# asarigun/mma

Hardware: AMD Instinct MI355X
Metric: aggregated edges/sec (fwd+bwd) MultiMaskConv (higher is better)
Workload: dtype f32

## Files before the change

### include/mma_amd.h

```cpp
#ifndef MMA_AMD_H
#define MMA_AMD_H

#include <stdint.h>

#ifdef __cplusplus
extern "C" {
#endif

#define MMA_ABI_VERSION 40
#define MMA_MAX_K 8

enum {
  MMA_KIND_SUM = 0,
  MMA_KIND_MEAN = 1,
  MMA_KIND_MAX = 2,
  MMA_KIND_MIN = 3,
  MMA_KIND_SOFTMAX = 4,
  MMA_KIND_SOFTMIN = 5
};
enum { MMA_ACT_SIGMOID = 0, MMA_ACT_RAW = 1 };

enum { MMA_DROP_NONE = 0, MMA_DROP_HASH = 1, MMA_DROP_EXPLICIT = 2 };

int mma_abi_version(void);
// ... 161 lines not shown
int mma_gemm_f16x2_k256p_h(const void* Ap, const int32_t* sce, const void* Bt2, const float* col_unscale, uint16_t* C, int64_t ldc,
                           int64_t M, int32_t N, void* stream);
int mma_gemm_f16x2_n128(const float* A, int64_t lda, const float* row_max, const void* Bt2, const float* col_unscale,
                        float* C, int64_t ldc, int64_t M, int32_t K, int32_t accumulate, void* stream);
int mma_gemm_f16x2_nlp(const float* A, int64_t lda, const float* row_max, const void* Bt2, const float* col_unscale,
                       float* C, int64_t ldc, int64_t M, int32_t N, int32_t K, int32_t accumulate, void* stream);
int64_t mma_gemm_bf16x3_tn_workspace_floats(int64_t M, int32_t KA, int32_t NC);
int mma_gemm_bf16x3_tn(const float* X, int64_t ldx, const float* G, int64_t ldg, float* C, float* ws, int64_t ws_floats,
                       int64_t M, int32_t KA, int32_t NC, void* stream);
int64_t mma_gemm_bf16x3_tn_batched_workspace_floats(int64_t M, int32_t KA, int32_t NC, int32_t B);
int mma_gemm_bf16x3_tn_batched(const float* X, int64_t ldx, int64_t xb, const float* G, int64_t ldg, int64_t gb, float* C, float* ws,
                               int64_t ws_floats, int64_t M, int32_t KA, int32_t NC, int32_t B, void* stream);
int64_t mma_gemm_f16x2_tn_workspace_floats(int64_t M, int32_t KA, int32_t NC);
int mma_gemm_f16x2_tn(const float* X, int64_t ldx, const float* G, int64_t ldg, const float* x_row_max, const float* g_row_max,
                      float* C, float* ws, int64_t ws_floats, int64_t M, int32_t KA, int32_t NC, void* stream);

int mma_pack_rows(const float* src, int64_t lds, const int32_t* idx, int64_t n_idx,
                  float* dst, int64_t ldd, int32_t width, void* stream);
int mma_unpack_add_rows(const float* src, int64_t lds, const int32_t* idx, int64_t n_idx,
                        float* dst, int64_t ldd, int32_t width, void* stream);
int mma_unpack_add_rows_csr(const float* src, int64_t lds, const int32_t* rows, const int32_t* segptr, const int32_t* pos,
                            int64_t n_rows, float* dst, int64_t ldd, int32_t width, void* stream);

int64_t mma_col_sum_workspace_floats(int64_t R, int32_t C);
int mma_col_sum(const float* g, int64_t ldg, int64_t R, int32_t C, float* out, float* ws, int64_t ws_floats,
                void* stream);

int64_t mma_tower_linear_bwd_blocks(int64_t N);
int mma_tower_linear_bwd(const float* gy, const float* a, const float* W, float* ga, float* part, int64_t n_blocks,
                         int64_t N, int32_t T, int32_t O, int32_t C, void* stream);
// ... 103 lines not shown
```

### mma_amd/_abi.py

```python
ABI_VERSION = 40
FUNCTIONS = {
    "mma_abi_version": ("int", []),
    "mma_last_error": ("const char*", []),
    "mma_build_stamp": ("const char*", []),
    "mma_nc_fused_fwd": ("int", [("T", "T", "x"), ("i", "i64", "ldx"), ("T", "T", "P"), ("i", "i64", "ldp"), ("T", "T", "Q"), ("i", "i64", "ldq"), ("T", "T", "rowptr"), ("T", "T", "col"), ("T", "T", "items"), ("i", "i64", "n_items"), ("i", "i64", "n_wave_items"), ("T", "T", "hubs"), ("i", "i64", "n_hubs"), ("T", "T", "partial"), ("i", "i64", "n_slots"), ("T", "T", "m"), ("T", "T", "m_sum"), ("i", "i64", "ldms"), ("T", "T", "T"), ("T", "T", "sel"), ("i", "i64", "ldt"), ("T", "T", "crow"), ("i", "i64", "ldc"), ("i", "i64", "N"), ("i", "i64", "E"), ("i", "i32", "H"), ("i", "i32", "K"), ("H", "H", "kind_host"), ("H", "H", "act_host"), ("i", "i32", "drop_mode"), ("i", "u32", "drop_thr"), ("i", "u64", "seed"), ("T", "T", "seed_dev"), ("i", "i64", "drop_edge_base"), ("T", "T", "keep"), ("T", "T", "sync"), ("S", "S", "stream")]),
    "mma_nc_bwd_node": ("int", [("T", "T", "g"), ("i", "i64", "g_kstride"), ("i", "i64", "ldgr"), ("T", "T", "sel"), ("T", "T", "T"), ("i", "i64", "ldt"), ("T", "T", "rowptr"), ("T", "T", "gs"), ("i", "i64", "ldgs"), ("T", "T", "crow"), ("i", "i64", "ldc"), ("T", "T", "gP"), ("i", "i64", "ldgp"), ("T", "T", "gxs"), ("i", "i64", "ldgx"), ("T", "T", "row_max"), ("i", "i64", "N"), ("i", "i32", "H"), ("i", "i32", "K"), ("H", "H", "kind_host"), ("S", "S", "stream")]),
    "mma_nc_crow_floats": ("int64_t", [("i", "i32", "H"), ("i", "i32", "K"), ("H", "H", "kind_host")]),
    "mma_nc_fused_bwd": ("int", [("T", "T", "x"), ("i", "i64", "ldx"), ("T", "T", "P"), ("i", "i64", "ldp"), ("T", "T", "Q"), ("i", "i64", "ldq"), ("T", "T", "gs"), ("i", "i64", "ldg"), ("T", "T", "g"), ("i", "i64", "ldgg"), ("T", "T", "crow"), ("i", "i64", "ldc"), ("H", "H", "kind_host"), ("T", "T", "gxs"), ("i", "i64", "ldgx"), ("T", "T", "T"), ("i", "i64", "ldt"), ("T", "T", "gP"), ("i", "i64", "ldgp"), ("i", "i64", "n_targets"), ("T", "T", "t_col"), ("T", "T", "t_eid"), ("T", "T", "items"), ("i", "i64", "n_items"), ("i", "i64", "n_wave_items"), ("T", "T", "hubs"), ("i", "i64", "n_hubs"), ("T", "T", "partial"), ("i", "i64", "n_slots"), ("T", "T", "gQ"), ("i", "i64", "ldgq"), ("T", "T", "gx"), ("i", "i64", "ldgxo"), ("T", "T", "row_max"), ("i", "i64", "N"), ("i", "i64", "E"), ("i", "i32", "H"), ("i", "i32", "K"), ("H", "H", "act_host"), ("i", "i32", "drop_mode"), ("i", "u32", "drop_thr"), ("i", "u64", "seed"), ("T", "T", "seed_dev"), ("i", "i64", "drop_edge_base"), ("T", "T", "keep"), ("T", "T", "sync"), ("S", "S", "stream")]),
    "mma_nc_fused_fwd_h": ("int", [("T", "T", "x"), ("i", "i64", "ldx"), ("T", "T", "P"), ("i", "i64", "ldp"), ("T", "T", "Q"), ("i", "i64", "ldq"), ("T", "T", "rowptr"), ("T", "T", "col"), ("T", "T", "items"), ("i", "i64", "n_items"), ("i", "i64", "n_wave_items"), ("T", "T", "hubs"), ("i", "i64", "n_hubs"), ("T", "T", "partial"), ("i", "i64", "n_slots"), ("T", "T", "m"), ("T", "T", "m_sum"), ("i", "i64", "ldms"), ("T", "T", "T"), ("T", "T", "sel"), ("i", "i64", "ldt"), ("T", "T", "crow"), ("i", "i64", "ldc"), ("i", "i64", "N"), ("i", "i64", "E"), ("i", "i32", "H"), ("i", "i32", "K"), ("H", "H", "kind_host"), ("H", "H", "act_host"), ("i", "i32", "drop_mode"), ("i", "u32", "drop_thr"), ("i", "u64", "seed"), ("T", "T", "seed_dev"), ("i", "i64", "drop_edge_base"), ("T", "T", "keep"), ("T", "T", "sync"), ("S", "S", "stream")]),
    "mma_nc_fused_bwd_h": ("int", [("T", "T", "x"), ("i", "i64", "ldx"), ("T", "T", "P"), ("i", "i64", "ldp"), ("T", "T", "Q"), ("i", "i64", "ldq"), ("T", "T", "gs"), ("i", "i64", "ldg"), ("T", "T", "g"), ("i", "i64", "ldgg"), ("T", "T", "crow"), ("i", "i64", "ldc"), ("H", "H", "kind_host"), ("T", "T", "gxs"), ("i", "i64", "ldgx"), ("T", "T", "T"), ("i", "i64", "ldt"), ("T", "T", "gP"), ("i", "i64", "ldgp"), ("i", "i64", "n_targets"), ("T", "T", "t_col"), ("T", "T", "t_eid"), ("T", "T", "items"), ("i", "i64", "n_items"), ("i", "i64", "n_wave_items"), ("T", "T", "hubs"), ("i", "i64", "n_hubs"), ("T", "T", "partial"), ("i", "i64", "n_slots"), ("T", "T", "gQ"), ("i", "i64", "ldgq"), ("T", "T", "gx"), ("i", "i64", "ldgxo"), ("T", "T", "row_max"), ("i", "i64", "N"), ("i", "i64", "E"), ("i", "i32", "H"), ("i", "i32", "K"), ("H", "H", "act_host"), ("i", "i32", "drop_mode"), ("i", "u32", "drop_thr"), ("i", "u64", "seed"), ("T", "T", "seed_dev"), ("i", "i64", "drop_edge_base"), ("T", "T", "keep"), ("T", "T", "sync"), ("S", "S", "stream")]),
    "mma_rows_to_bf16": ("int", [("T", "T", "src"), ("i", "i64", "lds"), ("T", "T", "dst"), ("i", "i64", "ldd"), ("i", "i64", "rows"), ("i", "i64", "cols"), ("S", "S", "stream")]),
    "mma_nc_std_fwd": ("int", [("T", "T", "x"), ("i", "i64", "ldx"), ("T", "T", "P"), ("i", "i64", "ldp"), ("T", "T", "Q"), ("i", "i64", "ldq"), ("T", "T", "rowptr"), ("T", "T", "col"), ("T", "T", "items"), ("i", "i64", "n_items"), ("i", "i64", "n_wave_items"), ("T", "T", "hubs"), ("i", "i64", "n_hubs"), ("T", "T", "partial"), ("i", "i64", "n_slots"), ("T", "T", "m"), ("i", "i64", "ldms"), ("T", "T", "saved"), ("i", "i64", "ldt"), ("i", "i64", "N"), ("i", "i64", "E"), ("i", "i32", "H"), ("H", "H", "act_host"), ("i", "i32", "drop_mode"), ("i", "u32", "drop_thr"), ("i", "u64", "seed"), ("T", "T", "seed_dev"), ("i", "i64", "drop_edge_base"), ("T", "T", "keep"), ("S", "S", "stream")]),
    "mma_nc_std_bwd": ("int", [("T", "T", "x"), ("i", "i64", "ldx"), ("T", "T", "P"), ("i", "i64", "ldp"), ("T", "T", "Q"), ("i", "i64", "ldq"), ("T", "T", "g"), ("i", "i64", "ldg"), ("T", "T", "saved"), ("i", "i64", "ldt"), ("T", "T", "gr"), ("i", "i64", "ldgr"), ("T", "T", "gP"), ("i", "i64", "ldgp"), ("i", "i64", "n_targets"), ("T", "T", "t_col"), ("T", "T", "t_eid"), ("T", "T", "items"), ("i", "i64", "n_items"), ("i", "i64", "n_wave_items"), ("T", "T", "hubs"), ("i", "i64", "n_hubs"), ("T", "T", "partial"), ("i", "i64", "n_slots"), ("T", "T", "gQ"), ("i", "i64", "ldgq"), ("T", "T", "gx"), ("i", "i64", "ldgx"), ("i", "i64", "N"), ("i", "i64", "E"), ("i", "i32", "H"), ("H", "H", "act_host"), ("i", "i32", "drop_mode"), ("i", "u32", "drop_thr"), ("i", "u64", "seed"), ("T", "T", "seed_dev"), ("i", "i64", "drop_edge_base"), ("T", "T", "keep"), ("S", "S", "stream")]),
    "mma_nc_std_fwd_h": ("int", [("T", "T", "x"), ("i", "i64", "ldx"), ("T", "T", "P"), ("i", "i64", "ldp"), ("T", "T", "Q"), ("i", "i64", "ldq"), ("T", "T", "rowptr"), ("T", "T", "col"), ("T", "T", "items"), ("i", "i64", "n_items"), ("i", "i64", "n_wave_items"), ("T", "T", "hubs"), ("i", "i64", "n_hubs"), ("T", "T", "partial"), ("i", "i64", "n_slots"), ("T", "T", "m"), ("i", "i64", "ldms"), ("T", "T", "saved"), ("i", "i64", "ldt"), ("i", "i64", "N"), ("i", "i64", "E"), ("i", "i32", "H"), ("H", "H", "act_host"), ("i", "i32", "drop_mode"), ("i", "u32", "drop_thr"), ("i", "u64", "seed"), ("T", "T", "seed_dev"), ("i", "i64", "drop_edge_base"), ("T", "T", "keep"), ("S", "S", "stream")]),
    "mma_nc_std_bwd_h": ("int", [("T", "T", "x"), ("i", "i64", "ldx"), ("T", "T", "P"), ("i", "i64", "ldp"), ("T", "T", "Q"), ("i", "i64", "ldq"), ("T", "T", "g"), ("i", "i64", "ldg"), ("T", "T", "saved"), ("i", "i64", "ldt"), ("T", "T", "gr"), ("i", "i64", "ldgr"), ("T", "T", "gP"), ("i", "i64", "ldgp"), ("i", "i64", "n_targets"), ("T", "T", "t_col"), ("T", "T", "t_eid"), ("T", "T", "items"), ("i", "i64", "n_items"), ("i", "i64", "n_wave_items"), ("T", "T", "hubs"), ("i", "i64", "n_hubs"), ("T", "T", "partial"), ("i", "i64", "n_slots"), ("T", "T", "gQ"), ("i", "i64", "ldgq"), ("T", "T", "gx"), ("i", "i64", "ldgx"), ("i", "i64", "N"), ("i", "i64", "E"), ("i", "i32", "H"), ("H", "H", "act_host"), ("i", "i32", "drop_mode"), ("i", "u32", "drop_thr"), ("i", "u64", "seed"), ("T", "T", "seed_dev"), ("i", "i64", "drop_edge_base"), ("T", "T", "keep"), ("S", "S", "stream")]),
    "mma_csr_spmm": ("int", [("T", "T", "rowptr"), ("T", "T", "col"), ("T", "T", "val"), ("T", "T", "B"), ("i", "i64", "ldb"), ("i", "i64", "rows_per_block"), ("i", "i32", "K"), ("T", "T", "bias"), ("T", "T", "out"), ("i", "i64", "ldo"), ("i", "i64", "n_rows"), ("i", "i32", "C"), ("S", "S", "stream")]),
    "mma_csr_spmm_rm": ("int", [("T", "T", "rowptr"), ("T", "T", "col"), ("T", "T", "val"), ("T", "T", "B"), ("i", "i64", "ldb"), ("i", "i64", "rows_per_block"), ("i", "i32", "K"), ("T", "T", "bias"), ("T", "T", "out"), ("i", "i64", "ldo"), ("i", "i64", "n_rows"), ("i", "i32", "C"), ("T", "T", "row_max"), ("S", "S", "stream")]),
    "mma_csr_spmm_items": ("int", [("T", "T", "col"), ("T", "T", "val"), ("T", "T", "B"), ("i", "i64", "ldb"), ("T", "T", "bias"), ("T", "T", "out"), ("i", "i64", "ldo"), ("T", "T", "items"), ("i", "i64", "n_items"), ("i", "i64", "n_wave_items"), ("T", "T", "hubs"), ("i", "i64", "n_hubs"), ("T", "T", "partial"), ("i", "i64", "n_slots"), ("i", "i32", "C"), ("S", "S", "stream")]),
    "mma_split_bf16x3": ("int", [("T", "T", "in"), ("i", "i64", "n"), ("T", "T", "out_3n_bf16"), ("S", "S", "stream")]),
    "mma_gemm_bf16x3": ("int", [("T", "T", "A"), ("i", "i64", "lda"), ("T", "T", "Bt3"), ("T", "T", "C"), ("i", "i64", "ldc"), ("i", "i64", "M"), ("i", "i32", "N"), ("i", "i32", "K"), ("i", "i32", "accumulate"), ("S", "S", "stream")]),
    "mma_row_absmax": ("int", [("T", "T", "A"), ("i", "i64", "lda"), ("i", "i64", "M"), ("i", "i32", "cols"), ("T", "T", "out"), ("S", "S", "stream")]),
    "mma_split_f16x2": ("int", [("T", "T", "w"), ("i", "i64", "stride_k"), ("i", "i64", "stride_n"), ("i", "i32", "K"), ("i", "i32", "N"), ("T", "T", "bt2"), ("T", "T", "col_unscale"), ("i", "i32", "plain_lo"), ("S", "S", "stream")]),
    "mma_gemm_f16x2": ("int", [("T", "T", "A"), ("i", "i64", "lda"), ("T", "T", "Bt2"), ("T", "T", "col_unscale"), ("T", "T", "C"), ("i", "i64", "ldc"), ("T", "T", "a_row_max"), ("i", "i64", "M"), ("i", "i32", "N"), ("S", "S", "stream")]),
    "mma_gemm_f16x2_k": ("int", [("T", "T", "A"), ("i", "i64", "lda"), ("T", "T", "Bt2"), ("T", "T", "col_unscale"), ("T", "T", "C"), ("i", "i64", "ldc"), ("T", "T", "a_row_max"), ("i", "i64", "M"), ("i", "i32", "N"), ("i", "i32", "K"), ("S", "S", "stream")]),
    "mma_gemm_f16x2_k256": ("int", [("T", "T", "A"), ("i", "i64", "lda"), ("T", "T", "row_max"), ("T", "T", "Bt2"), ("T", "T", "col_unscale"), ("T", "T", "C"), ("i", "i64", "ldc"), ("i", "i64", "M"), ("i", "i32", "N"), ("S", "S", "stream")]),
    "mma_pack_f16x2_k256_bytes": ("int64_t", [("i", "i64", "M")]),
    "mma_pack_f16x2_k256": ("int", [("T", "T", "A"), ("i", "i64", "lda"), ("i", "i64", "M"), ("T", "T", "Ap"), ("T", "T", "sce"), ("T", "T", "row_max"), ("S", "S", "stream")]),
    "mma_gemm_f16x2_k256p": ("int", [("T", "T", "Ap"), ("T", "T", "sce"), ("T", "T", "Bt2"), ("T", "T", "col_unscale"), ("T", "T", "C"), ("i", "i64", "ldc"), ("i", "i64", "M"), ("i", "i32", "N"), ("S", "S", "stream")]),
    "mma_gemm_f16x2_k_h": ("int", [("T", "T", "A"), ("i", "i64", "lda"), ("T", "T", "Bt2"), ("T", "T", "col_unscale"), ("T", "T", "C"), ("i", "i64", "ldc"), ("T", "T", "a_row_max"), ("i", "i64", "M"), ("i", "i32", "N"), ("i", "i32", "K"), ("S", "S", "stream")]),
    "mma_gemm_f16x2_k256_h": ("int", [("T", "T", "A"), ("i", "i64", "lda"), ("T", "T", "row_max"), ("T", "T", "Bt2"), ("T", "T", "col_unscale"), ("T", "T", "C"), ("i", "i64", "ldc"), ("i", "i64", "M"), ("i", "i32", "N"), ("S", "S", "stream")]),
    "mma_gemm_f16x2_k256p_h": ("int", [("T", "T", "Ap"), ("T", "T", "sce"), ("T", "T", "Bt2"), ("T", "T", "col_unscale"), ("T", "T", "C"), ("i", "i64", "ldc"), ("i", "i64", "M"), ("i", "i32", "N"), ("S", "S", "stream")]),
    "mma_gemm_f16x2_n128": ("int", [("T", "T", "A"), ("i", "i64", "lda"), ("T", "T", "row_max"), ("T", "T", "Bt2"), ("T", "T", "col_unscale"), ("T", "T", "C"), ("i", "i64", "ldc"), ("i", "i64", "M"), ("i", "i32", "K"), ("i", "i32", "accumulate"), ("S", "S", "stream")]),
    "mma_gemm_f16x2_nlp": ("int", [("T", "T", "A"), ("i", "i64", "lda"), ("T", "T", "row_max"), ("T", "T", "Bt2"), ("T", "T", "col_unscale"), ("T", "T", "C"), ("i", "i64", "ldc"), ("i", "i64", "M"), ("i", "i32", "N"), ("i", "i32", "K"), ("i", "i32", "accumulate"), ("S", "S", "stream")]),
    "mma_gemm_bf16x3_tn_workspace_floats": ("int64_t", [("i", "i64", "M"), ("i", "i32", "KA"), ("i", "i32", "NC")]),
    "mma_gemm_bf16x3_tn": ("int", [("T", "T", "X"), ("i", "i64", "ldx"), ("T", "T", "G"), ("i", "i64", "ldg"), ("T", "T", "C"), ("T", "T", "ws"), ("i", "i64", "ws_floats"), ("i", "i64", "M"), ("i", "i32", "KA"), ("i", "i32", "NC"), ("S", "S", "stream")]),
    "mma_gemm_bf16x3_tn_batched_workspace_floats": ("int64_t", [("i", "i64", "M"), ("i", "i32", "KA"), ("i", "i32", "NC"), ("i", "i32", "B")]),
    "mma_gemm_bf16x3_tn_batched": ("int", [("T", "T", "X"), ("i", "i64", "ldx"), ("i", "i64", "xb"), ("T", "T", "G"), ("i", "i64", "ldg"), ("i", "i64", "gb"), ("T", "T", "C"), ("T", "T", "ws"), ("i", "i64", "ws_floats"), ("i", "i64", "M"), ("i", "i32", "KA"), ("i", "i32", "NC"), ("i", "i32", "B"), ("S", "S", "stream")]),
    "mma_gemm_f16x2_tn_workspace_floats": ("int64_t", [("i", "i64", "M"), ("i", "i32", "KA"), ("i", "i32", "NC")]),
    "mma_gemm_f16x2_tn": ("int", [("T", "T", "X"), ("i", "i64", "ldx"), ("T", "T", "G"), ("i", "i64", "ldg"), ("T", "T", "x_row_max"), ("T", "T", "g_row_max"), ("T", "T", "C"), ("T", "T", "ws"), ("i", "i64", "ws_floats"), ("i", "i64", "M"), ("i", "i32", "KA"), ("i", "i32", "NC"), ("S", "S", "stream")]),
    "mma_pack_rows": ("int", [("T", "T", "src"), ("i", "i64", "lds"), ("T", "T", "idx"), ("i", "i64", "n_idx"), ("T", "T", "dst"), ("i", "i64", "ldd"), ("i", "i32", "width"), ("S", "S", "stream")]),
    "mma_unpack_add_rows": ("int", [("T", "T", "src"), ("i", "i64", "lds"), ("T", "T", "idx"), ("i", "i64", "n_idx"), ("T", "T", "dst"), ("i", "i64", "ldd"), ("i", "i32", "width"), ("S", "S", "stream")]),
    "mma_unpack_add_rows_csr": ("int", [("T", "T", "src"), ("i", "i64", "lds"), ("T", "T", "rows"), ("T", "T", "segptr"), ("T", "T", "pos"), ("i", "i64", "n_rows"), ("T", "T", "dst"), ("i", "i64", "ldd"), ("i", "i32", "width"), ("S", "S", "stream")]),
    "mma_col_sum_workspace_floats": ("int64_t", [("i", "i64", "R"), ("i", "i32", "C")]),
    "mma_col_sum": ("int", [("T", "T", "g"), ("i", "i64", "ldg"), ("i", "i64", "R"), ("i", "i32", "C"), ("T", "T", "out"), ("T", "T", "ws"), ("i", "i64", "ws_floats"), ("S", "S", "stream")]),
    "mma_tower_linear_bwd_blocks": ("int64_t", [("i", "i64", "N")]),
    "mma_tower_linear_bwd": ("int", [("T", "T", "gy"), ("T", "T", "a"), ("T", "T", "W"), ("T", "T", "ga"), ("T", "T", "part"), ("i", "i64", "n_blocks"), ("i", "i64", "N"), ("i", "i32", "T"), ("i", "i32", "O"), ("i", "i32", "C"), ("S", "S", "stream")]),
    "mma_tower_post_kfp": ("int64_t", [("i", "i32", "KF")]),
    "mma_tower_post_weights": ("int", [("T", "T", "Wo"), ("i", "i32", "T"), ("i", "i32", "O"), ("i", "i32", "S"), ("i", "i32", "KF"), ("T", "T", "Wa"), ("T", "T", "Wb"), ("S", "S", "stream")]),
    "mma_skinny_linear_weights": ("int", [("T", "T", "W"), ("i", "i32", "O"), ("i", "i32", "K"), ("T", "T", "Wa"), ("T", "T", "Wb"), ("S", "S", "stream")]),
    "mma_tower_post_gw_reduce": ("int", [("T", "T", "part"), ("i", "i64", "n_chunks"), ("i", "i32", "T"), ("i", "i32", "S"), ("i", "i32", "O"), ("i", "i32", "KF"), ("T", "T", "gWo"), ("S", "S", "stream")]),
    "mma_tower_post_fits": ("int", [("i", "i32", "KF"), ("i", "i32", "S")]),
    "mma_tower_post_pre": ("int", [("T", "T", "rowptr"), ("T", "T", "pre"), ("i", "i64", "N"), ("i", "i32", "S"), ("H", "H", "scaler_host"), ("f", "f32", "avg_log"), ("f", "f32", "avg_lin"), ("S", "S", "stream")]),
    "mma_tower_post_fwd": ("int", [("T", "T", "agg"), ("i", "i64", "lda"), ("T", "T", "pre"), ("T", "T", "Wa"), ("T", "T", "y"), ("i", "i64", "ldy"), ("i", "i64", "N"), ("i", "i32", "T"), ("i", "i32", "KF"), ("i", "i32", "S"), ("i", "i32", "O"), ("H", "H", "scaler_host"), ("f", "f32", "avg_log"), ("f", "f32", "avg_lin"), ("S", "S", "stream")]),
    "mma_tower_post_bwd": ("int", [("T", "T", "gy"), ("i", "i64", "ldg"), ("T", "T", "pre"), ("T", "T", "Wb"), ("T", "T", "gagg"), ("i", "i64", "lda"), ("T", "T", "gys"), ("i", "i64", "ldgs"), ("i", "i64", "N"), ("i", "i32", "T"), ("i", "i32", "KF"), ("i", "i32", "S"), ("i", "i32", "O"), ("H", "H", "scaler_host"), ("f", "f32", "avg_log"), ("f", "f32", "avg_lin"), ("S", "S", "stream")]),
# ... 30 lines not shown
```

### mma_amd/csrc/gemm_x3.hip

```cpp
#include <algorithm>
#include <cstdlib>
#include "common.h"

#ifndef MMA_ABL
#define MMA_ABL 0
#endif

namespace mma {

constexpr int kAbl = MMA_ABL;

typedef __attribute__((ext_vector_type(8))) __bf16 bf16x8;
typedef __attribute__((ext_vector_type(16))) float f32x16;

constexpr int kKC = 128;
constexpr int kKCPersist = 64;
struct GemmParams {
  const float* A; int64_t lda;
  const __bf16* Bt;
  float* C; int64_t ldc;
  int64_t M; int N, K;
  int accumulate;
};

// ... 1254 lines not shown
  if (wave_active) {
    float* out = p.part + (size_t)split * (p.part_ss ? (size_t)p.part_ss : (size_t)p.KA * p.NC) + (size_t)bz * p.KA * p.NC +
                 (size_t)wave * 32 * p.NC + gcol0 + r31;
#pragma unroll
    for (int ct = 0; ct < 4; ++ct) {
      if (ct < n_ct) {
#pragma unroll
        for (int r = 0; r < 16; ++r)
          if (FULLCT || (wave * 32 + acc_row(r) + 4 * h < p.KA && gcol0 + ct * 32 + r31 < p.NC))
            out[(size_t)(acc_row(r) + 4 * h) * p.NC + ct * 32] = acc[ct][r];
      }
    }
  }
}

typedef __attribute__((ext_vector_type(4))) unsigned int u32x4;
constexpr int kTn2Slab = 2 * kTnPiece;
constexpr int kTnMaxSpread = 40;

__global__ void tn_state_init_kernel(int* state) {
  if (threadIdx.x < 4) state[threadIdx.x] = 0;
}

__global__ __launch_bounds__(256) void tn_scale_range_kernel(const float* xmax, const float* gmax, int64_t M, int* state) {
  __shared__ int red[3][4];
  int hi = 0, lo = 0, bad = 0;
  for (int64_t i = (int64_t)blockIdx.x * blockDim.x + threadIdx.x; i < M; i += (int64_t)gridDim.x * blockDim.x) {
    const uint32_t xb = __float_as_uint(xmax[i]) & 0x7fffffffu, gb = __float_as_uint(gmax[i]) & 0x7fffffffu;
    if (xb != 0 && gb != 0) {
      const int ex = (int)(xb >> 23), eg = (int)(gb >> 23);
      if (ex == 255 || eg == 255 || ex == 0 || eg == 0) bad = 1;
      else { const int t = ex + eg - 254; hi = max(hi, t + 1024); lo = max(lo, 1024 - t); }
    }
  }
#pragma unroll
  for (int o = 32; o > 0; o >>= 1) {
    hi = max(hi, __shfl_xor(hi, o, 64)); lo = max(lo, __shfl_xor(lo, o, 64)); bad |= __shfl_xor(bad, o, 64);
  }
  const int wave = threadIdx.x >> 6;
  if ((threadIdx.x & 63) == 0) { red[0][wave] = hi; red[1][wave] = lo; red[2][wave] = bad; }
  __syncthreads();
  if (threadIdx.x == 0) {
    hi = max(max(red[0][0], red[0][1]), max(red[0][2], red[0][3]));
    lo = max(max(red[1][0], red[1][1]), max(red[1][2], red[1][3]));
    bad = red[2][0] | red[2][1] | red[2][2] | red[2][3];
    if (hi) atomicMax(state + 0, hi);
    if (lo) atomicMax(state + 1, lo);
    if (bad) atomicOr(state + 2, 1);
  }
}

__global__ void tn_scale_rows_kernel(const float* xmax, const float* gmax, int64_t M, int64_t M_pad, int* state, uint16_t* sxh,
                                     uint16_t* sgh) {
  const int64_t i = (int64_t)blockIdx.x * blockDim.x + threadIdx.x;
  const int T = state[0] ? state[0] - 1024 : 28;
  if (i == 0) state[3] = T - 28;
  const uint32_t xb = i < M ? __float_as_uint(xmax[i]) & 0x7fffffffu : 0u, gb = i < M ? __float_as_uint(gmax[i]) & 0x7fffffffu : 0u;
  uint16_t hx = 0, hg = 0;
  bool bad = false;
  if (xb != 0 && gb != 0) {
    const int ex = (int)(xb >> 23) - 127, eg = (int)(gb >> 23) - 127;
    const int r = T - (ex + eg);
    const int px = 14 - ex - (r >> 1), pg = 14 - eg - (r - (r >> 1));
    bad = r > kTnMaxSpread || px < -126 || px > 127 || pg < -126 || pg > 127;
    if (!bad) { hx = (uint16_t)((px + 127) << 7); hg = (uint16_t)((pg + 127) << 7); }
  }
  if (__any(bad) && (threadIdx.x & 63) == 0 && state[2] == 0) atomicOr(state + 2, 1);
  if (i < M_pad) { sxh[i] = hx; sgh[i] = hg; }
}

template <bool VEC>
// ... 270 lines not shown
  return kGo;
}
#define MMA_CHECKED(call) do { if (const int rc_ = (call); rc_ != kGo) return rc_; } while (0)

struct TnPlan { int64_t rps; dim3 grid; };
static int tn_plan(int s, int64_t M, int64_t ldx, int64_t ldg, int NC, int B, TnPlan& pl) {
  pl.rps = ((M + s - 1) / s + kTnKC - 1) / kTnKC * kTnKC;
  MMA_REQUIRE((pl.rps + kTnKC) * (ldx > ldg ? ldx : ldg) * 4 < (1LL << 31), "row range of one split exceeds a 2 GB buffer window");
  pl.grid = dim3((unsigned)(((NC + 127) / 128) * s), (unsigned)B);
  return kGo;
}
static void launch_x3_tn(const TnParams& p, dim3 grid, hipStream_t st) {
  if (p.NC % 128 == 0 && p.KA % 32 == 0) hipLaunchKernelGGL(gemm_x3_tn_kernel<true>, grid, dim3(kBlock), 0, st, p);
  else hipLaunchKernelGGL(gemm_x3_tn_kernel<false>, grid, dim3(kBlock), 0, st, p);
}
template <int NW>
static void launch_f16x2_tn(const TnParams& p, dim3 grid, hipStream_t st, bool full, bool px) {
  if (px && full) hipLaunchKernelGGL((gemm_f16x2_tn_kernel<true, NW, true>), grid, dim3(64 * NW), 0, st, p);
  else if (px) hipLaunchKernelGGL((gemm_f16x2_tn_kernel<false, NW, true>), grid, dim3(64 * NW), 0, st, p);
  else if (full) hipLaunchKernelGGL((gemm_f16x2_tn_kernel<true, NW>), grid, dim3(64 * NW), 0, st, p);
  else hipLaunchKernelGGL((gemm_f16x2_tn_kernel<false, NW>), grid, dim3(64 * NW), 0, st, p);
}

extern "C" int mma_split_bf16x3(const float* in, int64_t n, void* out, void* stream) {
  MMA_REQUIRE(n >= 0, "n < 0");
  if (n == 0) return 0;
  MMA_REQUIRE(in && out, "NULL argument");
  int64_t blocks = (n + kBlock - 1) / kBlock;
  if (blocks > kMaxGrid) blocks = kMaxGrid;
  hipLaunchKernelGGL(split3_kernel, dim3((unsigned)blocks), dim3(kBlock), 0, static_cast<hipStream_t>(stream), in, n,
// ... 205 lines not shown

extern "C" int mma_col_sum(const float* g, int64_t ldg, int64_t R, int32_t C, float* out, float* ws, int64_t ws_floats, void* stream);

extern "C" int mma_gemm_bf16x3_tn(const float* X, int64_t ldx, const float* G, int64_t ldg, float* C, float* ws, int64_t ws_floats,
                                  int64_t M, int32_t KA, int32_t NC, void* stream) {
  MMA_REQUIRE(M >= 1 && KA >= 1 && KA <= 128 && NC >= 1 && (int64_t)KA * NC < (1LL << 31), "M=%lld KA=%d NC=%d: need 1 <= KA <= 128, NC >= 1",
              (long long)M, KA, NC);
  MMA_REQUIRE(X && G && C && ldx >= KA && ldg >= NC && ldx < (1 << 24) && ldg < (1 << 24), "NULL argument or row pitch out of range");
  MMA_REQUIRE((reinterpret_cast<uintptr_t>(X) & 3) == 0 && (reinterpret_cast<uintptr_t>(G) & 3) == 0, "misaligned argument");
  const int s = tn_splits(M, NC);
  MMA_REQUIRE(s == 1 || (ws && ws_floats >= (int64_t)s * KA * NC), "workspace too small: %lld floats, need %lld",
              (long long)ws_floats, (long long)s * KA * NC);
  TnPlan pl;
  MMA_CHECKED(tn_plan(s, M, ldx, ldg, NC, 1, pl));
  TnParams p{X, ldx, G, ldg, s == 1 ? C : ws, M, pl.rps, KA, NC, s};
  launch_x3_tn(p, pl.grid, static_cast<hipStream_t>(stream));
  if (int rc = check_launch("gemm_x3_tn_kernel")) return rc;
  if (s == 1) return 0;
  return mma_col_sum(ws, (int64_t)KA * NC, s, KA * NC, C, nullptr, 0, stream);
}

static int tn_splits_batched(int64_t M, int NC, int B) {
  const int64_t n_cb = ((int64_t)NC + 127) / 128;
  int64_t s = 512 / (n_cb * B);
  const int64_t max_s = M / (8 * kTnKC) + 1;
  if (s > max_s) s = max_s;
  if (s >= 8) s = s / 8 * 8;
  return (int)(s < 1 ? 1 : s);
}
extern "C" int64_t mma_gemm_bf16x3_tn_batched_workspace_floats(int64_t M, int32_t KA, int32_t NC, int32_t B) {
  if (M <= 0 || KA <= 0 || NC <= 0 || B <= 0) return 0;
// ... 28 lines not shown
  MMA_REQUIRE(A && out && (reinterpret_cast<uintptr_t>(A) & 3) == 0, "NULL or misaligned argument");
  launch_row_absmax(A, lda, M, cols, out, static_cast<hipStream_t>(stream));
  return check_launch("row_absmax_kernel");
}

static bool tn_packx(int64_t M, int KA, int NC) {
  const char* e = getenv("MMA_TN_PACKX");
  if (e && (e[0] == '0' || e[0] == '1')) return e[0] == '1';
  return M >= 65536 && ((int64_t)NC + 127) / 128 >= 16;
}
static int64_t tn_packx_floats(int64_t M, int KA) { return tn_pad32(M) / 32 * (((int64_t)KA + 31) / 32) * 1024; }

extern "C" int64_t mma_gemm_f16x2_tn_workspace_floats(int64_t M, int32_t KA, int32_t NC) {
  if (M <= 0 || KA <= 0 || NC <= 0) return 0;
  const int s = tn_splits(M, NC);
  return (s > 1 ? ((int64_t)s * KA * NC + 3) / 4 * 4 : 0) + 3 * tn_pad32(M) + 4 + (tn_packx(M, KA, NC) ? tn_packx_floats(M, KA) : 0);
}

extern "C" int mma_gemm_f16x2_tn(const float* X, int64_t ldx, const float* G, int64_t ldg, const float* x_row_max, const float* g_row_max,
                                 float* C, float* ws, int64_t ws_floats, int64_t M, int32_t KA, int32_t NC, void* stream) {
  MMA_REQUIRE(M >= 1 && M < (1LL << 30) && KA >= 1 && KA <= 256 && NC >= 1 && (int64_t)KA * NC < (1LL << 31),
              "M=%lld KA=%d NC=%d: need M < 2^30, 1 <= KA <= 256, NC >= 1", (long long)M, KA, NC);
  MMA_REQUIRE(X && G && C && ws && ldx >= KA && ldg >= NC && ldx < (1 << 24) && ldg < (1 << 24), "NULL argument or row pitch out of range");
  MMA_REQUIRE((reinterpret_cast<uintptr_t>(X) & 3) == 0 && (reinterpret_cast<uintptr_t>(G) & 3) == 0 &&
              (reinterpret_cast<uintptr_t>(ws) & 15) == 0, "misaligned argument");
  const int s = tn_splits(M, NC);
  const int64_t n_part = s > 1 ? ((int64_t)s * KA * NC + 3) / 4 * 4 : 0, Mp = tn_pad32(M);
  const bool px = tn_packx(M, KA, NC);
  const int64_t n_need = n_part + 3 * Mp + 4 + (px ? tn_packx_floats(M, KA) : 0);
  MMA_REQUIRE(ws_floats >= n_need, "workspace too small: %lld floats, need %lld", (long long)ws_floats, (long long)n_need);
  TnPlan pl;
  MMA_CHECKED(tn_plan(s, M, ldx, ldg, NC, 1, pl));
  const int64_t rps = pl.rps;
  const dim3 grid = pl.grid;
  const int nb = (KA + 31) / 32;
  MMA_REQUIRE(!px || (rps / kTnKC + 1) * (int64_t)nb * 4096 < (1LL << 31), "packed rows of one split exceed a 2 GB buffer window");
  float* xmax = ws + n_part;
  float* gmax = xmax + Mp;
  uint16_t* sxh = reinterpret_cast<uint16_t*>(gmax + Mp);
  uint16_t* sgh = sxh + Mp;
  int* state = reinterpret_cast<int*>(gmax + 2 * Mp);
  hipStream_t st = static_cast<hipStream_t>(stream);
  hipLaunchKernelGGL(tn_state_init_kernel, dim3(1), dim3(64), 0, st, state);
  if (!x_row_max) { launch_row_absmax(X, ldx, M, KA, xmax, st); x_row_max = xmax; }
  if (!g_row_max) { launch_row_absmax(G, ldg, M, NC, gmax, st); g_row_max = gmax; }
  hipLaunchKernelGGL(tn_scale_range_kernel, dim3((unsigned)std::min<int64_t>((M + 255) / 256, 256)), dim3(256), 0, st, x_row_max, g_row_max, M,
                     state);
  hipLaunchKernelGGL(tn_scale_rows_kernel, dim3((unsigned)((Mp + 255) / 256)), dim3(256), 0, st, x_row_max, g_row_max, M, Mp, state, sxh, sgh);
  if (int rc = check_launch("tn_scale_rows_kernel")) return rc;
  TnParams p{X, ldx, G, ldg, s == 1 ? C : ws, M, rps, KA, NC, s, sxh, sgh, state, 0};
  const bool full = NC % 128 == 0 && KA % 32 == 0;
  if (px) {
    u32x4* xp = reinterpret_cast<u32x4*>(ws + n_part + 3 * Mp + 4);
    const int64_t n_items = Mp / 32 * nb;
    hipLaunchKernelGGL(tn_pack_x_kernel, dim3((unsigned)std::min<int64_t>((n_items + 3) / 4, 8 * 2048)), dim3(256), 0, st, X, ldx, M, (int)KA, sxh,
                       xp, nb, n_items);
    p.xp = xp; p.xp_nb = nb;
  }
  if (KA > 128) launch_f16x2_tn<8>(p, grid, st, full, px);
  else launch_f16x2_tn<4>(p, grid, st, full, px);
  p.want_bad = 1;
  for (int j = 0; j < KA; j += 128) {
    TnParams q = p;
    q.X = X + j; q.KA = KA - j < 128 ? KA - j : 128;
    q.part = p.part + (size_t)j * NC; q.part_ss = (int64_t)KA * NC;
    launch_x3_tn(q, grid, st);
  }
  if (int rc = check_launch("gemm_f16x2_tn_kernel")) return rc;
  if (s == 1) return 0;
  return mma_col_sum(ws, (int64_t)KA * NC, s, KA * NC, C, nullptr, 0, stream);
}
```

### mma_amd/dense.py

```python
from functools import partial

import torch

from . import _lib
from ._env import flag, integer
from ._lib import call, ptr, stream_ptr


def _span(name, nbytes=0, flops=0, mfma=None):
    from . import functional as Fn
    return Fn._span(name, nbytes, flops, mfma)

_ROWS_PER_BATCH = 8192
_MIN_ROWS_X3 = 4096
_MIN_COLS_TN = integer("MMA_MIN_COLS_TN", 1)
_MIN_ROWS_TN = integer("MMA_MIN_ROWS_TN", 1024)
_MIN_ROWS_F16X2 = 1 << 16
USE_F16X2 = True
F16X2_K = (64, 96, 128)
PACK_K256 = flag("MMA_PACK_K256")
USE_NLP = flag("MMA_DX_NLP")
TN_KA256 = flag("MMA_TN_KA256")
BF16_EPILOGUE = flag("MMA_BF16_EPILOGUE")
_BF16_OUT_FORMS = ("f16x2_k", "f16x2_k256", "f16x2_k256p")
# ... 33 lines not shown
            _lib.query("mma_gemm_bf16x3_tn_batched_workspace_floats", M, KA, NC, batch))
    splits = max(1, n_ws // ((batch or 1) * KA * NC))
    rows = -(-(-(-M // splits)) // 32) * 32
    return (rows + 32) * pitch * 4 < 2 ** 31


def tn_form(M, KA, NC, *, ldx, ldg, g_row_max_known=False, batch=None, named=False):
    pitch = max(ldx, ldg)
    if (batch is not None and M >= _MIN_ROWS_X3 and 8 <= KA <= 128 and NC >= 32 and pitch < (1 << 24)
            and _tn_window_fits(M, KA, NC, pitch, batch)):
        return "bf16x3_tn_batched"
    if not named and not (M >= _MIN_ROWS_TN and (8 <= KA <= 128 or KA % 128 == 0) and NC >= _MIN_COLS_TN
                          and _tn_window_fits(M, min(KA, 128), NC, pitch)):
        return "lib"
    return "f16x2_tn" if USE_F16X2 and g_row_max_known and M >= _MIN_ROWS_F16X2 else "bf16x3_tn"


def _gpu_f32(*ts, unit_cols=False, aligned=False):
    return all(t.is_cuda and t.dtype == torch.float32 and (not (unit_cols or aligned) or t.stride(1) == 1)
               and (not aligned or (t.stride(0) % 4 == 0 and t.data_ptr() % 16 == 0)) for t in ts)


def _gemm_span(name, mfma, M, K, N, accumulate=False, c_bytes=4):
    return _span(name, nbytes=M * (4 * K + c_bytes * (2 if accumulate else 1) * N), flops=2 * M * K * N, mfma=mfma)


def _c_suffix(out):
    if out.dtype not in (torch.float32, torch.bfloat16):
        raise ValueError("the three-product column-group GEMMs write float32 or bfloat16, but got %r" % (out.dtype,))
    return ("", 4) if out.dtype == torch.float32 else ("_h", 2)
# ... 497 lines not shown
```

Before: 768.1 million.

## Add narrow-NC bf16x3 TN GEMM kernel and drop state-init launch via per-block slots

Adds a dedicated bf16x3 TN GEMM kernel for NC<=32 and KA<=128. It runs one 32-wide MFMA tile per wave with double-buffered LDS and buffer loads prefetched three chunks ahead, instead of the general kernel whose tiles waste work on narrow outputs. It also replaces the atomic-based scale-range reduction with per-block slots that the scale-rows kernel reduces, which removes the separate state-init kernel launch, and unrolls the range loop by four. The narrow path can be turned off with an env var, and the workspace grows by the slot storage.

```diff
diff --git a/include/mma_amd.h b/include/mma_amd.h
--- a/include/mma_amd.h
+++ b/include/mma_amd.h
@@ -7,7 +7,7 @@
 extern "C" {
 #endif
 
-#define MMA_ABI_VERSION 40
+#define MMA_ABI_VERSION 41
 #define MMA_MAX_K 8
 
 enum {
@@ -199,6 +199,7 @@
 int64_t mma_gemm_f16x2_tn_workspace_floats(int64_t M, int32_t KA, int32_t NC);
 int mma_gemm_f16x2_tn(const float* X, int64_t ldx, const float* G, int64_t ldg, const float* x_row_max, const float* g_row_max,
                       float* C, float* ws, int64_t ws_floats, int64_t M, int32_t KA, int32_t NC, void* stream);
+int mma_gemm_bf16x3_tn_narrow(int32_t KA, int32_t NC);
 
 int mma_pack_rows(const float* src, int64_t lds, const int32_t* idx, int64_t n_idx,
                   float* dst, int64_t ldd, int32_t width, void* stream);
diff --git a/mma_amd/_abi.py b/mma_amd/_abi.py
--- a/mma_amd/_abi.py
+++ b/mma_amd/_abi.py
@@ -1,4 +1,4 @@
-ABI_VERSION = 40
+ABI_VERSION = 41
 FUNCTIONS = {
     "mma_abi_version": ("int", []),
     "mma_last_error": ("const char*", []),
@@ -38,6 +38,7 @@
     "mma_gemm_bf16x3_tn_batched": ("int", [("T", "T", "X"), ("i", "i64", "ldx"), ("i", "i64", "xb"), ("T", "T", "G"), ("i", "i64", "ldg"), ("i", "i64", "gb"), ("T", "T", "C"), ("T", "T", "ws"), ("i", "i64", "ws_floats"), ("i", "i64", "M"), ("i", "i32", "KA"), ("i", "i32", "NC"), ("i", "i32", "B"), ("S", "S", "stream")]),
     "mma_gemm_f16x2_tn_workspace_floats": ("int64_t", [("i", "i64", "M"), ("i", "i32", "KA"), ("i", "i32", "NC")]),
     "mma_gemm_f16x2_tn": ("int", [("T", "T", "X"), ("i", "i64", "ldx"), ("T", "T", "G"), ("i", "i64", "ldg"), ("T", "T", "x_row_max"), ("T", "T", "g_row_max"), ("T", "T", "C"), ("T", "T", "ws"), ("i", "i64", "ws_floats"), ("i", "i64", "M"), ("i", "i32", "KA"), ("i", "i32", "NC"), ("S", "S", "stream")]),
+    "mma_gemm_bf16x3_tn_narrow": ("int", [("i", "i32", "KA"), ("i", "i32", "NC")]),
     "mma_pack_rows": ("int", [("T", "T", "src"), ("i", "i64", "lds"), ("T", "T", "idx"), ("i", "i64", "n_idx"), ("T", "T", "dst"), ("i", "i64", "ldd"), ("i", "i32", "width"), ("S", "S", "stream")]),
     "mma_unpack_add_rows": ("int", [("T", "T", "src"), ("i", "i64", "lds"), ("T", "T", "idx"), ("i", "i64", "n_idx"), ("T", "T", "dst"), ("i", "i64", "ldd"), ("i", "i32", "width"), ("S", "S", "stream")]),
     "mma_unpack_add_rows_csr": ("int", [("T", "T", "src"), ("i", "i64", "lds"), ("T", "T", "rows"), ("T", "T", "segptr"), ("T", "T", "pos"), ("i", "i64", "n_rows"), ("T", "T", "dst"), ("i", "i64", "ldd"), ("i", "i32", "width"), ("S", "S", "stream")]),
diff --git a/mma_amd/csrc/gemm_x3.hip b/mma_amd/csrc/gemm_x3.hip
--- a/mma_amd/csrc/gemm_x3.hip
+++ b/mma_amd/csrc/gemm_x3.hip
@@ -1292,23 +1292,134 @@
   }
 }
 
+typedef __attribute__((ext_vector_type(4))) __bf16 bf16x4;
+constexpr int kTnNPiece = 32 * kTnPitch;
+constexpr int kTnNSlab = 3 * kTnNPiece;
+
+__global__ __launch_bounds__(kBlock, 2) void gemm_x3_tn_narrow_kernel(const TnParams p) {
+  __shared__ __attribute__((aligned(16))) unsigned char lds[2 * kTnNSlab];
+  const int tid = threadIdx.x;
+  const int lane = tid & 63, wave = tid >> 6;
+  const int r31 = lane & 31, h = lane >> 5;
+  const int split = (int)blockIdx.x;
+  const int64_t r0 = (int64_t)split * p.rows_per_split;
+  const int64_t r1 = min(p.M, r0 + p.rows_per_split);
+  const int n_chunks = r1 > r0 ? (int)((r1 - r0 + kTnKC - 1) / kTnKC) : 0;
+  const bool wave_active = wave * 32 < p.KA;
+  const int sn = tid & 31, sq = tid >> 5;
+  const int scol = sn < p.NC ? sn : 0;
+  const int xcol = min(wave * 32 + r31, p.KA - 1);
+  const int ldg_b = (int)p.ldg * 4, ldx_b = (int)p.ldx * 4;
+  const int rows = (int)(r1 > r0 ? r1 - r0 : 0);
+  const int64_t rbase = r1 > r0 ? r0 : 0;
+  const auto g_rsrc = __builtin_amdgcn_make_buffer_rsrc(const_cast<float*>(p.G + rbase * p.ldg), 0, rows ? (rows - 1) * ldg_b + p.NC * 4 : 0,
+                                                        0x00020000);
+  const auto x_rsrc = __builtin_amdgcn_make_buffer_rsrc(const_cast<float*>(p.X + rbase * p.ldx), 0, rows ? (rows - 1) * ldx_b + p.KA * 4 : 0,
+                                                        0x00020000);
+  const int g_voff = sq * 4 * ldg_b + scol * 4;
+  const int x_voff = 8 * h * ldx_b + xcol * 4;
+
+  f32x16 acc;
+#pragma unroll
+  for (int r = 0; r < 16; ++r) acc[r] = 0.f;
+  float graw0[4], xraw0[16], graw1[4], xraw1[16];
+  bf16x8 af[2][3];
+
+#define MMA_TNN_LOAD(C_, GR_, XR_)                                                             \
+  {                                                                                            \
+    int gv = g_voff + (C_) * (kTnKC * ldg_b);                                                  \
+    int xv = x_voff + (C_) * (kTnKC * ldx_b);                                                  \
+    asm volatile("" : "+v"(gv), "+v"(xv));                                                     \
+    _Pragma("unroll") for (int i = 0; i < 4; ++i)                                              \
+      GR_[i] = __uint_as_float(__builtin_amdgcn_raw_buffer_load_b32(g_rsrc, gv + i * ldg_b, 0, 0)); \
+    _Pragma("unroll") for (int ks = 0; ks < 2; ++ks)                                           \
+      _Pragma("unroll") for (int i = 0; i < 8; ++i)                                            \
+        XR_[ks * 8 + i] = __uint_as_float(__builtin_amdgcn_raw_buffer_load_b32(x_rsrc, xv + (ks * 16 + i) * ldx_b, 0, 0)); \
+  }
+#define MMA_TNN_PUBLISH_G(B_, GR_)                                                             \
+  {                                                                                            \
+    bf16x4 a, b, c;                                                                            \
+    _Pragma("unroll") for (int i = 0; i < 4; ++i) {                                            \
+      const Bf3 t = split3(GR_[i]);                                                            \
+      a[i] = t.a; b[i] = t.b; c[i] = t.c;                                                      \
+    }                                                                                          \
+    unsigned char* d = lds + (B_) * kTnNSlab + sn * kTnPitch + sq * 8;                         \
+    *reinterpret_cast<bf16x4*>(d + 0 * kTnNPiece) = a;                                         \
+    *reinterpret_cast<bf16x4*>(d + 1 * kTnNPiece) = b;                                         \
+    *reinterpret_cast<bf16x4*>(d + 2 * kTnNPiece) = c;                                         \
+  }
+#define MMA_TNN_STEP(C_, B_, GR_, XR_)                                                         \
+  {                                                                                            \
+    const unsigned char* sb = lds + (B_) * kTnNSlab + r31 * kTnPitch + h * 16;                 \
+    bf16x8 bq[2][3];                                                                           \
+    _Pragma("unroll") for (int ks = 0; ks < 2; ++ks)                                           \
+      _Pragma("unroll") for (int q = 0; q < 3; ++q)                                            \
+        bq[ks][q] = *reinterpret_cast<const bf16x8*>(sb + ks * 32 + q * kTnNPiece);            \
+    _Pragma("unroll") for (int ks = 0; ks < 2; ++ks) {                                         \
+      acc = __builtin_amdgcn_mfma_f32_32x32x16_bf16(af[ks][0], bq[ks][2], acc, 0, 0, 0);       \
+      acc = __builtin_amdgcn_mfma_f32_32x32x16_bf16(af[ks][1], bq[ks][1], acc, 0, 0, 0);       \
+      acc = __builtin_amdgcn_mfma_f32_32x32x16_bf16(af[ks][2], bq[ks][0], acc, 0, 0, 0);       \
+      acc = __builtin_amdgcn_mfma_f32_32x32x16_bf16(af[ks][0], bq[ks][1], acc, 0, 0, 0);       \
+      acc = __builtin_amdgcn_mfma_f32_32x32x16_bf16(af[ks][1], bq[ks][0], acc, 0, 0, 0);       \
+      acc = __builtin_amdgcn_mfma_f32_32x32x16_bf16(af[ks][0], bq[ks][0], acc, 0, 0, 0);       \
+      if (ks == 0) MMA_TNN_PUBLISH_G(1 - (B_), GR_)                                            \
+      __builtin_amdgcn_sched_barrier(0);                                                       \
+    }                                                                                          \
+    _Pragma("unroll") for (int ks = 0; ks < 2; ++ks) split3x8(XR_, ks * 8, af[ks][0], af[ks][1], af[ks][2]); \
+    MMA_TNN_LOAD((C_) + 3, GR_, XR_)                                                           \
+    asm volatile("s_waitcnt lgkmcnt(0)" ::: "memory");                                         \
+    __builtin_amdgcn_s_barrier();                                                              \
+    asm volatile("" ::: "memory");                                                             \
+  }
+
+  MMA_TNN_LOAD(0, graw0, xraw0)
+  MMA_TNN_PUBLISH_G(0, graw0)
+#pragma unroll
+  for (int ks = 0; ks < 2; ++ks) split3x8(xraw0, ks * 8, af[ks][0], af[ks][1], af[ks][2]);
+  MMA_TNN_LOAD(1, graw1, xraw1)
+  MMA_TNN_LOAD(2, graw0, xraw0)
+  __syncthreads();
+  for (int c = 0; c < n_chunks; c += 2) {
+    MMA_TNN_STEP(c, 0, graw1, xraw1)
+    MMA_TNN_STEP(c + 1, 1, graw0, xraw0)
+  }
+#undef MMA_TNN_STEP
+#undef MMA_TNN_PUBLISH_G
+#undef MMA_TNN_LOAD
+
+  if (wave_active) {
+    float* out = p.part + (size_t)split * p.KA * p.NC + (size_t)wave * 32 * p.NC + r31;
+#pragma unroll
+    for (int r = 0; r < 16; ++r)
+      if (wave * 32 + acc_row(r) + 4 * h < p.KA && r31 < p.NC) out[(size_t)(acc_row(r) + 4 * h) * p.NC] = acc[r];
+  }
+}
+
 typedef __attribute__((ext_vector_type(4))) unsigned int u32x4;
 constexpr int kTn2Slab = 2 * kTnPiece;
 constexpr int kTnMaxSpread = 40;
 
-__global__ void tn_state_init_kernel(int* state) {
-  if (threadIdx.x < 4) state[threadIdx.x] = 0;
-}
+constexpr int kTnRangeBlocks = 256;
+constexpr int kTnStateInts = 4 + 3 * kTnRangeBlocks;
 
 __global__ __launch_bounds__(256) void tn_scale_range_kernel(const float* xmax, const float* gmax, int64_t M, int* state) {
   __shared__ int red[3][4];
   int hi = 0, lo = 0, bad = 0;
-  for (int64_t i = (int64_t)blockIdx.x * blockDim.x + threadIdx.x; i < M; i += (int64_t)gridDim.x * blockDim.x) {
-    const uint32_t xb = __float_as_uint(xmax[i]) & 0x7fffffffu, gb = __float_as_uint(gmax[i]) & 0x7fffffffu;
-    if (xb != 0 && gb != 0) {
-      const int ex = (int)(xb >> 23), eg = (int)(gb >> 23);
-      if (ex == 255 || eg == 255 || ex == 0 || eg == 0) bad = 1;
-      else { const int t = ex + eg - 254; hi = max(hi, t + 1024); lo = max(lo, 1024 - t); }
+  const int64_t stride = (int64_t)gridDim.x * blockDim.x;
+  for (int64_t i = (int64_t)blockIdx.x * blockDim.x + threadIdx.x; i < M; i += 4 * stride) {
+    uint32_t xb[4], gb[4];
+#pragma unroll
+    for (int k = 0; k < 4; ++k) {
+      const int64_t j = i + k * stride < M ? i + k * stride : i;
+      xb[k] = __float_as_uint(xmax[j]) & 0x7fffffffu; gb[k] = __float_as_uint(gmax[j]) & 0x7fffffffu;
+    }
+#pragma unroll
+    for (int k = 0; k < 4; ++k) {
+      if (i + k * stride < M && xb[k] != 0 && gb[k] != 0) {
+        const int ex = (int)(xb[k] >> 23), eg = (int)(gb[k] >> 23);
+        if (ex == 255 || eg == 255 || ex == 0 || eg == 0) bad = 1;
+        else { const int t = ex + eg - 254; hi = max(hi, t + 1024); lo = max(lo, 1024 - t); }
+      }
     }
   }
 #pragma unroll
@@ -1322,17 +1433,33 @@
     hi = max(max(red[0][0], red[0][1]), max(red[0][2], red[0][3]));
     lo = max(max(red[1][0], red[1][1]), max(red[1][2], red[1][3]));
     bad = red[2][0] | red[2][1] | red[2][2] | red[2][3];
-    if (hi) atomicMax(state + 0, hi);
-    if (lo) atomicMax(state + 1, lo);
-    if (bad) atomicOr(state + 2, 1);
-  }
-}
-
-__global__ void tn_scale_rows_kernel(const float* xmax, const float* gmax, int64_t M, int64_t M_pad, int* state, uint16_t* sxh,
-                                     uint16_t* sgh) {
+    int* slot = state + 4 + 3 * blockIdx.x;
+    slot[0] = hi; slot[1] = lo; slot[2] = bad;
+    if (blockIdx.x == 0) state[2] = 0;
+  }
+}
+
+__global__ __launch_bounds__(256) void tn_scale_rows_kernel(const float* xmax, const float* gmax, int64_t M, int64_t M_pad, int* state,
+                                                            int n_slots, uint16_t* sxh, uint16_t* sgh) {
   const int64_t i = (int64_t)blockIdx.x * blockDim.x + threadIdx.x;
-  const int T = state[0] ? state[0] - 1024 : 28;
-  if (i == 0) state[3] = T - 28;
+  __shared__ int red[3][4];
+  int s_hi = 0, s_lo = 0, s_bad = 0;
+  for (int s = threadIdx.x; s < n_slots; s += 256) {
+    const int* slot = state + 4 + 3 * s;
+    s_hi = max(s_hi, slot[0]); s_lo = max(s_lo, slot[1]); s_bad |= slot[2];
+  }
+#pragma unroll
+  for (int o = 32; o > 0; o >>= 1) {
+    s_hi = max(s_hi, __shfl_xor(s_hi, o, 64)); s_lo = max(s_lo, __shfl_xor(s_lo, o, 64)); s_bad |= __shfl_xor(s_bad, o, 64);
+  }
+  if ((threadIdx.x & 63) == 0) { red[0][threadIdx.x >> 6] = s_hi; red[1][threadIdx.x >> 6] = s_lo; red[2][threadIdx.x >> 6] = s_bad; }
+  __syncthreads();
+  s_hi = max(max(red[0][0], red[0][1]), max(red[0][2], red[0][3]));
+  const int T = s_hi ? s_hi - 1024 : 28;
+  if (i == 0) {
+    state[0] = s_hi; state[1] = max(max(red[1][0], red[1][1]), max(red[1][2], red[1][3])); state[3] = T - 28;
+    if (red[2][0] | red[2][1] | red[2][2] | red[2][3]) atomicOr(state + 2, 1);
+  }
   const uint32_t xb = i < M ? __float_as_uint(xmax[i]) & 0x7fffffffu : 0u, gb = i < M ? __float_as_uint(gmax[i]) & 0x7fffffffu : 0u;
   uint16_t hx = 0, hg = 0;
   bool bad = false;
@@ -1633,6 +1760,10 @@
   if (p.NC % 128 == 0 && p.KA % 32 == 0) hipLaunchKernelGGL(gemm_x3_tn_kernel<true>, grid, dim3(kBlock), 0, st, p);
   else hipLaunchKernelGGL(gemm_x3_tn_kernel<false>, grid, dim3(kBlock), 0, st, p);
 }
+static bool tn_narrow(int KA, int NC) {
+  const char* e = getenv("MMA_TN_NARROW");
+  return NC <= 32 && KA <= 128 && !(e && e[0] == '0');
+}
 template <int NW>
 static void launch_f16x2_tn(const TnParams& p, dim3 grid, hipStream_t st, bool full, bool px) {
   if (px && full) hipLaunchKernelGGL((gemm_f16x2_tn_kernel<true, NW, true>), grid, dim3(64 * NW), 0, st, p);
@@ -1868,7 +1999,8 @@
   TnPlan pl;
   MMA_CHECKED(tn_plan(s, M, ldx, ldg, NC, 1, pl));
   TnParams p{X, ldx, G, ldg, s == 1 ? C : ws, M, pl.rps, KA, NC, s};
-  launch_x3_tn(p, pl.grid, static_cast<hipStream_t>(stream));
+  if (tn_narrow(KA, NC)) hipLaunchKernelGGL(gemm_x3_tn_narrow_kernel, pl.grid, dim3(kBlock), 0, static_cast<hipStream_t>(stream), p);
+  else launch_x3_tn(p, pl.grid, static_cast<hipStream_t>(stream));
   if (int rc = check_launch("gemm_x3_tn_kernel")) return rc;
   if (s == 1) return 0;
   return mma_col_sum(ws, (int64_t)KA * NC, s, KA * NC, C, nullptr, 0, stream);
@@ -1927,7 +2059,7 @@
 extern "C" int64_t mma_gemm_f16x2_tn_workspace_floats(int64_t M, int32_t KA, int32_t NC) {
   if (M <= 0 || KA <= 0 || NC <= 0) return 0;
   const int s = tn_splits(M, NC);
-  return (s > 1 ? ((int64_t)s * KA * NC + 3) / 4 * 4 : 0) + 3 * tn_pad32(M) + 4 + (tn_packx(M, KA, NC) ? tn_packx_floats(M, KA) : 0);
+  return (s > 1 ? ((int64_t)s * KA * NC + 3) / 4 * 4 : 0) + 3 * tn_pad32(M) + kTnStateInts + (tn_packx(M, KA, NC) ? tn_packx_floats(M, KA) : 0);
 }
 
 extern "C" int mma_gemm_f16x2_tn(const float* X, int64_t ldx, const float* G, int64_t ldg, const float* x_row_max, const float* g_row_max,
@@ -1940,7 +2072,7 @@
   const int s = tn_splits(M, NC);
   const int64_t n_part = s > 1 ? ((int64_t)s * KA * NC + 3) / 4 * 4 : 0, Mp = tn_pad32(M);
   const bool px = tn_packx(M, KA, NC);
-  const int64_t n_need = n_part + 3 * Mp + 4 + (px ? tn_packx_floats(M, KA) : 0);
+  const int64_t n_need = n_part + 3 * Mp + kTnStateInts + (px ? tn_packx_floats(M, KA) : 0);
   MMA_REQUIRE(ws_floats >= n_need, "workspace too small: %lld floats, need %lld", (long long)ws_floats, (long long)n_need);
   TnPlan pl;
   MMA_CHECKED(tn_plan(s, M, ldx, ldg, NC, 1, pl));
@@ -1954,17 +2086,17 @@
   uint16_t* sgh = sxh + Mp;
   int* state = reinterpret_cast<int*>(gmax + 2 * Mp);
   hipStream_t st = static_cast<hipStream_t>(stream);
-  hipLaunchKernelGGL(tn_state_init_kernel, dim3(1), dim3(64), 0, st, state);
   if (!x_row_max) { launch_row_absmax(X, ldx, M, KA, xmax, st); x_row_max = xmax; }
   if (!g_row_max) { launch_row_absmax(G, ldg, M, NC, gmax, st); g_row_max = gmax; }
-  hipLaunchKernelGGL(tn_scale_range_kernel, dim3((unsigned)std::min<int64_t>((M + 255) / 256, 256)), dim3(256), 0, st, x_row_max, g_row_max, M,
-                     state);
-  hipLaunchKernelGGL(tn_scale_rows_kernel, dim3((unsigned)((Mp + 255) / 256)), dim3(256), 0, st, x_row_max, g_row_max, M, Mp, state, sxh, sgh);
+  const int n_slots = (int)std::min<int64_t>((M + 255) / 256, kTnRangeBlocks);
+  hipLaunchKernelGGL(tn_scale_range_kernel, dim3((unsigned)n_slots), dim3(256), 0, st, x_row_max, g_row_max, M, state);
+  hipLaunchKernelGGL(tn_scale_rows_kernel, dim3((unsigned)((Mp + 255) / 256)), dim3(256), 0, st, x_row_max, g_row_max, M, Mp, state, n_slots, sxh,
+                     sgh);
   if (int rc = check_launch("tn_scale_rows_kernel")) return rc;
   TnParams p{X, ldx, G, ldg, s == 1 ? C : ws, M, rps, KA, NC, s, sxh, sgh, state, 0};
   const bool full = NC % 128 == 0 && KA % 32 == 0;
   if (px) {
-    u32x4* xp = reinterpret_cast<u32x4*>(ws + n_part + 3 * Mp + 4);
+    u32x4* xp = reinterpret_cast<u32x4*>(ws + n_part + 3 * Mp + kTnStateInts);
     const int64_t n_items = Mp / 32 * nb;
     hipLaunchKernelGGL(tn_pack_x_kernel, dim3((unsigned)std::min<int64_t>((n_items + 3) / 4, 8 * 2048)), dim3(256), 0, st, X, ldx, M, (int)KA, sxh,
                        xp, nb, n_items);
@@ -1983,3 +2115,5 @@
   if (s == 1) return 0;
   return mma_col_sum(ws, (int64_t)KA * NC, s, KA * NC, C, nullptr, 0, stream);
 }
+
+extern "C" int mma_gemm_bf16x3_tn_narrow(int32_t KA, int32_t NC) { return KA >= 1 && NC >= 1 && tn_narrow(KA, NC) ? 1 : 0; }
diff --git a/mma_amd/dense.py b/mma_amd/dense.py
--- a/mma_amd/dense.py
+++ b/mma_amd/dense.py
@@ -71,6 +71,10 @@
                           and _tn_window_fits(M, min(KA, 128), NC, pitch)):
         return "lib"
     return "f16x2_tn" if USE_F16X2 and g_row_max_known and M >= _MIN_ROWS_F16X2 else "bf16x3_tn"
+
+
+def tn_narrow(form, KA, NC):
+    return form == "bf16x3_tn" and bool(_lib.query("mma_gemm_bf16x3_tn_narrow", min(KA, 128), NC))
 
 
 def _gpu_f32(*ts, unit_cols=False, aligned=False):
```

New measurement: 770.6 million, median of 6. No clear change (+0.3%).
